# peterWon/GLoc3D

Hardware: AMD Instinct MI355X
Metric: localization queries/sec (kNN+top-20 reg), KITTI-00-sized DB (higher is better)
Workload: dtype f32

## Files before the change

gloc3d_amd/capi.py:

```python
import ctypes as C
import os

import numpy as np

HERE = os.path.dirname(os.path.abspath(__file__))
LIB_PATH = os.environ.get("GLOC3D_LIB_PATH") or os.path.join(HERE, "lib", "libgloc3d.so")

GLOC_OK = 0
ERR_NAMES = {1: "GLOC_ERR_INVALID", 2: "GLOC_ERR_HIP", 3: "GLOC_ERR_NOMEM", 4: "GLOC_ERR_NODEVICE",
             5: "GLOC_ERR_STATE"}
ALGO_AUTO, ALGO_EXACT, ALGO_MFMA, ALGO_MFMA_FP32 = 0, 1, 2, 3
KNN_OPT_ALGO, KNN_OPT_CANDIDATES, KNN_OPT_PROFILE = 1, 2, 3
REG_OPT_PROFILE, REG_OPT_NN_MODE, REG_OPT_NN_SRC_PER_LANE, REG_OPT_NN_JOB_GROUP, REG_OPT_TEMP_TARGET_INDEX = 1, 2, 3, 4, 5
REG_OPT_NN_SPLIT_HELPERS, REG_OPT_NN_SPLIT_THRESH, REG_OPT_NN_SUB_JOBS, REG_OPT_NN_HEAVY_THRESH, REG_OPT_SUB_BATCHES = 6, 7, 8, 9, 10
REG_OPT_NN_CHAIN = 11
REG_OPT_PAIRGRAPH_BUDGET = 12
REG_NN_CULLED, REG_NN_EXHAUSTIVE = 0, 1
NO_SCAN = 0xFFFFFFFF
SIZE_MAX = C.c_size_t(-1).value


class GlocError(RuntimeError):
    def __init__(self, code, msg):
        super().__init__(f"{ERR_NAMES.get(code, code)}: {msg}")
# ... 832 lines not shown
        perm, keys, kpos = np.empty(n, np.uint32), np.empty(n, np.uint32), np.empty(n, np.uint32)
        order2 = np.empty((n + 127) // 128, np.uint32)
        kd = C.c_int()
        check(f(self._h, int(scan_id), _np_ptr(perm), _np_ptr(keys), _np_ptr(kpos), _np_ptr(order2), C.byref(kd)))
        return dict(perm=perm, keys=keys, kpos=kpos, order2=order2, kd=bool(kd.value))

    def debug_boxes(self, scan_id, cs=2):
        f = lib().gloc_scan_store_debug_boxes
        f.restype = C.c_int
        f.argtypes = [C.c_void_p, C.c_uint32, C.c_int] + [C.c_void_p] * 9
        n = self.points(scan_id)
        nch = (n + 127) // 128
        n_pad, nsup, group = nch * 128, (nch + 63) // 64, 64 * int(cs)
        hb, hg = np.empty(6, np.uint32), np.empty(4, np.float32)
        box_lo, box_hi = np.empty((nch, 4), np.float32), np.empty((nch, 4), np.float32)
        sb2 = np.empty((n_pad // 32, 3, 4), np.float32)
        sup_lo, sup_hi = np.empty((nsup, 4), np.float32), np.empty((nsup, 4), np.float32)
        pad = np.empty((n_pad - n, 4), np.float32)
        order = np.empty((n + group - 1) // group if group else 0, np.uint32)
        check(f(self._h, int(scan_id), int(cs), *[_np_ptr(a) for a in (hb, hg, box_lo, box_hi, sb2, sup_lo, sup_hi, pad, order)]))
        return dict(lo=hb[:3].copy(), hi=hb[3:].copy(), ox=hg[0], oy=hg[1], oz=hg[2], inv_cell=hg[3], box_lo=box_lo,
                    box_hi=box_hi, sb2=sb2, sup_lo=sup_lo, sup_hi=sup_hi, pad=pad, order=order)

    def build_target_index_batch(self, scan_ids):
        ids = np.ascontiguousarray(scan_ids, np.uint32).reshape(-1)
        check(lib().gloc_scan_store_build_target_index_batch(self._h, _np_ptr(ids), ids.shape[0]))

    def release(self, scan_id):
        check(lib().gloc_scan_store_release(self._h, int(scan_id)))

    def clear(self):
        check(lib().gloc_scan_store_clear(self._h))

    def __len__(self):
        n = C.c_size_t()
        check(lib().gloc_scan_store_count(self._h, C.byref(n)))
        return n.value

    def bytes(self):
        a, b = C.c_size_t(), C.c_size_t()
        check(lib().gloc_scan_store_bytes(self._h, C.byref(a), C.byref(b)))
        return a.value, b.value

    def points(self, scan_id):
        n = C.c_size_t()
        check(lib().gloc_scan_store_points(self._h, int(scan_id), C.byref(n)))
# ... 1032 lines not shown
```

gloc3d_amd/csrc/nn_compact.hpp:

```cpp
#pragma once
#include <hip/hip_runtime.h>
#include <stdint.h>

#include <type_traits>

#include "lane_ops.hpp"
#include "reg_kernels.hpp"

namespace gloc {
namespace reg {

typedef float f32x2 __attribute__((ext_vector_type(2)));

#define GPTR(T) const T __attribute__((address_space(1)))*
#define CPTR(T) const T __attribute__((address_space(4)))*
constexpr float NN_NEAR = 1.0e-6f;
constexpr float NN_LB_SCALE = 0.999998f;
#ifndef GLOC_NN_THIN_MIN
#define GLOC_NN_THIN_MIN 32
#endif
#ifdef GLOC_NN_MARKS
#define NN_MARK(n) asm volatile("; NN_MARK " n)
#else
#define NN_MARK(n)
// ... 228 lines not shown
          uint32_t word = 0;
          if (parts > 1 && first + parts <= sp.hx) {
            for (uint32_t p = 0; p < parts; ++p) st_u32<true>(helper + first + p, g | (p << 20) | (parts << 24));
            word = (hid << 8) | parts;
          }
          st_u32<true>(plan + g, word);
        }
        run_h += 4u * (uint32_t)__popcll(b4) + 8u * (uint32_t)__popcll(b8);
        run_l += 2u * (uint32_t)__popcll(b2);
        run_gh += (uint32_t)__popcll(b4 | b8);
        run_gl += (uint32_t)__popcll(b2);
      }
    }
    for (uint32_t g = ng + (uint32_t)lane; g < n_groups; g += 64) st_u32<true>(plan + g, 0u);
  }
  if (pass + 1u < ch.n_pass) (void)chain_arrive(ch.ready + ((size_t)(pass + 1u) * n_jobs + job) * NN_CHAIN_PAD);
}


struct NnPos {
  uint32_t grp, slot, wgv;
  uint32_t role = 0, pass = 0, job = 0;
};

template <int CS, bool PAIRS, bool SPLIT = false ,
          bool WARM = false, bool HEAVY = false ,
          bool CHAIN = false >
__device__ __forceinline__ void nn_compact_body(
    const NnPos pos ,
    const Job* __restrict__ jobs, uint32_t n_jobs, uint32_t job_group, uint32_t n_wg , uint32_t subs,
    const CandState* __restrict__ states,
    const uint32_t* prev_corr , uint32_t* corr, float* __restrict__ d2out,
    f32x4* __restrict__ pairs, double* __restrict__ partials , uint32_t n_part,
    size_t ld, float gate2, NnSplit sp, NnHeavy hv, unsigned long long* __restrict__ stat_pairs ,
    const NnChain ch = NnChain{}) {
  constexpr int S = 64 * CS;
  constexpr int NSB = CH / SB;
  constexpr int SB_STRIDE = (SB / 2) * 8 + 8;
#ifndef GLOC_NN_QCAP
#define GLOC_NN_QCAP 256
#endif
#ifndef GLOC_NN_GRAN
#define GLOC_NN_GRAN 64
#endif
  constexpr int QCAP = GLOC_NN_QCAP;
  struct WaveLds {
// ... 53 lines not shown
    own_wave = false;
    if (gi >= J.n_groups) return;
  } else {
    const uint32_t wv = __builtin_amdgcn_readfirstlane(wg * NN_WPB + w);
    if (SPLIT && wv < sp.hx) {
      const uint32_t hw = ((CPTR(uint32_t))sp.helper)[(size_t)job * sp.hx + wv];
      if (hw == NN_NO_HELPER) return;
      gi = hw & 0xFFFFFu;
      part = (hw >> 20) & 15u;
      parts = hw >> 24;
      own_wave = false;
    } else {
      gi = wv - (SPLIT ? sp.hx : 0u);
    }
    if (gi >= J.n_groups) return;
    if constexpr (SPLIT) plan_word = ((CPTR(uint32_t))sp.plan)[(size_t)job * n_part + gi];
  }
  const unsigned long long pmask =
      !SPLIT || parts == 1 ? ~0ull : ((parts == 2 ? 0x5555555555555555ull : (parts == 4 ? 0x1111111111111111ull : (parts == 8 ? 0x0101010101010101ull : 0x0001000100010001ull))) << part);
  uint32_t w_cand = 0;
  struct IndexView {
    GPTR(f32x4) pts; GPTR(f32x4) box_lo; GPTR(f32x4) box_hi; GPTR(f32x4) sb2;
    GPTR(uint32_t) keys; GPTR(uint32_t) kpos; GPTR(uint32_t) inv; GPTR(ScanHeader) hdr;
    uint32_t n, nchunks;
    GPTR(f32x4) sup_lo; GPTR(f32x4) sup_hi;
    uint32_t nsup;
    CPTR(f32x4) cbox_lo; CPTR(f32x4) cbox_hi;
  };
  const ScanIndexDev ixg = J.tgt;
  const IndexView ix{(GPTR(f32x4))ixg.pts, (GPTR(f32x4))ixg.box_lo, (GPTR(f32x4))ixg.box_hi,
                     (GPTR(f32x4))ixg.sb2, (GPTR(uint32_t))ixg.keys, (GPTR(uint32_t))ixg.kpos,
                     (GPTR(uint32_t))ixg.inv, (GPTR(ScanHeader))ixg.hdr, ixg.n, ixg.nchunks,
                     (GPTR(f32x4))ixg.sup_lo, (GPTR(f32x4))ixg.sup_hi, ixg.nsup,
                     (CPTR(f32x4))ixg.box_lo, (CPTR(f32x4))ixg.box_hi};
  GPTR(f32x4) src4 = (GPTR(f32x4))J.src_pts;
  float T[12];
#pragma unroll
  for (int i = 0; i < 12; ++i) {
    if constexpr (CHAIN) T[i] = pos.pass ? ((CPTR(float))ch.Tp)[((size_t)pos.pass * n_jobs + job) * NN_CHAIN_T_STRIDE + i] : states[job].Tf[i];
    else T[i] = states[job].Tf[i];
  }

  const uint32_t wave_base = ((CPTR(uint32_t))J.src_order)[gi] * S;
  if constexpr (SPLIT && !HEAVY) {
    if (own_wave && (plan_word & 0xFFu) != 0u) return;
    hid = plan_word >> 8;
  }
  uint32_t n_processed = 0;
  unsigned long long n_items = 0;
  [[maybe_unused]] uint32_t n_rounds = 0;

  NN_MARK("load_xform_box");
  float px[CS], py[CS], pz[CS], best[CS];
  bool valid[CS];
  float wlo[3] = {3.4e38f, 3.4e38f, 3.4e38f}, whi[3] = {-3.4e38f, -3.4e38f, -3.4e38f};
// ... 30 lines not shown
  NN_MARK("upper_bounds");
  uint32_t b0s[CS];
#pragma unroll
  for (int s = 0; s < CS; ++s) {
    b0s[s] = 0;
    if (ix.n && pj[s] < ix.n) {
      const f32x4 t = pt[s];
      best[s] = dist2(px[s], py[s], pz[s], t.x, t.y, t.z);
      b0s[s] = pj[s] / (SB / 4);
    }
  }
  uint8_t tie0[CS];
#pragma unroll
  for (int s = 0; s < CS; ++s) tie0[s] = 0;
  if constexpr (HEAVY) {
#pragma unroll
    for (int s = 0; s < CS; ++s) {
      const unsigned long long k = hv.hkey[(size_t)hid * S + s * 64 + lane];
      best[s] = __uint_as_float((uint32_t)(k >> 32));
      b0s[s] = (uint32_t)k & 0x7FFFFFFFu;
      tie0[s] = (uint8_t)(((uint32_t)k >> 31) & 1u);
    }
  } else if constexpr (!WARM) {
#ifndef GLOC_NN_KEY_PROBES
#define GLOC_NN_KEY_PROBES 3
#endif
    constexpr int KP = GLOC_NN_KEY_PROBES;
    bool cold[CS];
    uint32_t key[CS], lo[CS], hi[CS];
    bool any = false;
#pragma unroll
    for (int s = 0; s < CS; ++s) {
      cold[s] = ix.n && !(pj[s] < ix.n);
      key[s] = morton_key(px[s], py[s], pz[s], ix.hdr->ox, ix.hdr->oy, ix.hdr->oz, ix.hdr->inv_cell);
      lo[s] = 0;
      hi[s] = cold[s] ? ix.n : 0u;
      any |= cold[s];
    }
    if (any) {
      for (;;) {
        bool go = false;
#pragma unroll
        for (int s = 0; s < CS; ++s) go |= hi[s] - lo[s] > (uint32_t)KP;
        if (!go) break;
        uint32_t pos[CS][KP], kv[CS][KP];
#pragma unroll
// ... 43 lines not shown
        for (int d = -2; d <= 2; ++d) {
          long long jj = (long long)lo[s] + d;
          jj = jj < 0 ? 0 : (jj >= (long long)ix.n ? (long long)ix.n - 1 : jj);
          pjj[s][d + 2] = !cold[s] ? 0u : (ix.kpos ? ix.kpos[jj] : (uint32_t)jj);
        }
      f32x4 tn[CS][5];
#pragma unroll
      for (int s = 0; s < CS; ++s)
#pragma unroll
        for (int d = 0; d < 5; ++d) tn[s][d] = ix.pts[pjj[s][d]];
#pragma unroll
      for (int s = 0; s < CS; ++s) {
        if (!cold[s]) continue;
#pragma unroll
        for (int d = 0; d < 5; ++d) {
          const float dd = dist2(px[s], py[s], pz[s], tn[s][d].x, tn[s][d].y, tn[s][d].z);
          if (dd < best[s]) {
            best[s] = dd;
            b0s[s] = pjj[s][d] / (SB / 4);
          }
        }
      }
    }
  }
#pragma unroll
  for (int s = 0; s < CS; ++s) {
    const uint32_t b0 = b0s[s];
    if (!valid[s]) best[s] = -1.f;
    const int slot = s * 64 + lane;
    L.src[slot] = f32x4{px[s], py[s], pz[s], 0.f};
    L.key[slot] = ((unsigned long long)__float_as_uint(best[s]) << 32) | b0;
    L.tie[slot] = tie0[s];
  }
  if (lane == 0) {
    L.src[S] = f32x4{0.f, 0.f, 0.f, 0.f};
    L.key[S] = (unsigned long long)__float_as_uint(-1.f) << 32;
  }
  constexpr float KS = SB2_INV_RANGE * SB2_INV_RANGE / NN_LB_SCALE;
  float bests[CS];
#pragma unroll
  for (int s = 0; s < CS; ++s) bests[s] = best[s] * KS;
  auto wave_max_best = [&]() {
    float m = -1.f;
#pragma unroll
    for (int s = 0; s < CS; ++s) m = fmaxf(m, bests[s]);
    return wave_minmax<true>(m);
// ... 244 lines not shown
            const unsigned long long k = L.key[slot];
            const unsigned long long old = __hip_atomic_fetch_min(hv.hkey + (size_t)hid * S + slot, k, __ATOMIC_RELAXED, __HIP_MEMORY_SCOPE_AGENT);
            const unsigned long long oldk = old & ~0x80000000ull;
            if (oldk < k) {
              const float od = __uint_as_float((uint32_t)(oldk >> 32)), md = __uint_as_float((uint32_t)(k >> 32));
              if ((old & 0x80000000ull) != 0ull || (md <= od * (1.0f + NN_NEAR) && ((uint32_t)oldk >> 2) != ((uint32_t)k >> 2))) L.tie[slot] = 1;
              L.key[slot] = oldk;
            }
          }
        }
      }
      bool changed = false;
#pragma unroll
      for (int s = 0; s < CS; ++s) {
        const float nb = __uint_as_float((uint32_t)(L.key[s * 64 + lane] >> 32));
        const float nbs = nb * KS;
        changed |= nbs < bests[s];
        bests[s] = nbs;
      }
      if (!WARM || wmax_s > 1.0e30f) {
        if (__builtin_amdgcn_ballot_w64(changed) != 0ull) wmax_s = wave_max_best();
      }
    };
  constexpr int NSEED = 4;
  uint32_t seed_c[NSEED];
#pragma unroll
  for (int k = 0; k < NSEED; ++k) seed_c[k] = 0xFFFFFFFFu;
  if constexpr (!WARM) {
    if (parts == 1 && ix.nchunks) {
      bool pend[CS];
      uint32_t sc[CS];
#pragma unroll
      for (int s = 0; s < CS; ++s) {
        sc[s] = b0s[s] / (uint32_t)(CH / (SB / 4));
        pend[s] = valid[s] && best[s] < 3.0e38f;
      }
      for (int k = 0; k < NSEED; ++k) {
        uint32_t c = 0xFFFFFFFFu;
#pragma unroll
        for (int s = CS - 1; s >= 0; --s) {
          const unsigned long long m = __builtin_amdgcn_ballot_w64(pend[s]);
          if (m) c = (uint32_t)__builtin_amdgcn_readlane((int)sc[s], __ffsll((long long)m) - 1);
        }
        if (c == 0xFFFFFFFFu) break;
        c = c < ix.nchunks ? c : ix.nchunks - 1;
#pragma unroll
        for (int j = 0; j < NSEED; ++j)
// ... 352 lines not shown
```

gloc3d_amd/csrc/scan_index.hpp:

```cpp
#pragma once
#include <hip/hip_runtime.h>
#include <stdint.h>

#include "math3.hpp"

namespace gloc {
namespace reg {

constexpr int CH = 128;
constexpr int SB = 16;
constexpr float SB2_RANGE = 64.f, SB2_INV_RANGE = 1.f / 64.f;

struct ScanHeader {
  float ox, oy, oz, inv_cell;
  uint32_t lo[3], hi[3];
  uint32_t pad_[6];
};
static_assert(sizeof(ScanHeader) == 64, "header is 64 bytes");

struct ScanIndexDev {
  const f32x4* pts;
  const f32x4* box_lo;
  const f32x4* box_hi;
  const f32x4* sb2;
  const uint32_t* kpos;
  const uint32_t* keys;
  const uint32_t* inv;
  const ScanHeader* hdr;
  const f32x4* sup_lo;
  const f32x4* sup_hi;
  uint32_t n, nchunks, nsup, pad_;
};

__host__ __device__ __forceinline__ uint32_t f2ord(float f) {
  const uint32_t u = __builtin_bit_cast(uint32_t, f);
  return (u & 0x80000000u) ? ~u : (u | 0x80000000u);
}
__host__ __device__ __forceinline__ float ord2f(uint32_t o) {
  const uint32_t u = (o & 0x80000000u) ? (o & 0x7FFFFFFFu) : ~o;
  return __builtin_bit_cast(float, u);
}

__host__ __device__ __forceinline__ bool finite_coord(float f) {
  return (__builtin_bit_cast(uint32_t, f) & 0x7F800000u) != 0x7F800000u;
}

}
}
```

gloc3d_amd/csrc/scan_store.hip:

```cpp
#include <algorithm>
#include <new>

#include "fpfh.hpp"
#include "scan_store.hpp"
#include "seg_sort.hpp"
#include <cmath>

#include "raycast_kernels.hpp"
#include "synth_kernels.hpp"

namespace gloc {
namespace reg {

constexpr int PACK_BLOCKS = 128;

struct ScanBuild {
  const float* in;
  ScanHeader* hdr;
  float* xyz;
  f32x4* pts;
  f32x4* lo;
  f32x4* hi;
  f32x4* sb2;
  f32x4* ulo;
// ... 264 lines not shown
                                    float sigma, uint64_t key, float* __restrict__ out) {
  const uint32_t i = blockIdx.x * blockDim.x + threadIdx.x;
  if (i >= n) return;
  float T[12];
#pragma unroll
  for (int k = 0; k < 12; ++k) T[k] = T12[k];
  float x, y, z;
  xform(T, xyz[3 * (size_t)i], xyz[3 * (size_t)i + 1], xyz[3 * (size_t)i + 2], x, y, z);
  const float nx = sigma * synth::rng_gauss(key, 3ull * i + 0);
  const float ny = sigma * synth::rng_gauss(key, 3ull * i + 1);
  const float nz = sigma * synth::rng_gauss(key, 3ull * i + 2);
  out[3 * (size_t)i + 0] = x + nx;
  out[3 * (size_t)i + 1] = y + ny;
  out[3 * (size_t)i + 2] = z + nz;
}

struct ScanKd {
  f32x4* pts;
  uint32_t* inv;
  uint32_t* kpos;
  uint32_t n, n_pad, levels;
  uint32_t off;
  uint32_t box_off;
  uint32_t pad_;
};

__global__ void kd_load_kernel(const ScanKd* __restrict__ ks, f32x4* __restrict__ p, uint32_t* __restrict__ h) {
  const ScanKd& k = ks[blockIdx.y];
  const uint32_t i = blockIdx.x * blockDim.x + threadIdx.x;
  if (i >= k.n) return;
  p[k.off + i] = k.pts[i];
  h[k.off + i] = i;
}

__global__ void kd_box_init_kernel(const ScanKd* __restrict__ ks, uint32_t level, uint32_t* __restrict__ box) {
  const ScanKd& k = ks[blockIdx.y];
  const uint32_t nd = blockIdx.x * blockDim.x + threadIdx.x;
  if (level >= k.levels || nd >= (1u << level)) return;
  uint32_t* b = box + k.box_off + 6 * (size_t)nd;
#pragma unroll
  for (int a = 0; a < 3; ++a) {
    b[a] = 0xFFFFFFFFu;
    b[3 + a] = 0u;
  }
}

__global__ __launch_bounds__(256) void kd_node_bbox_kernel(const ScanKd* __restrict__ ks, uint32_t level,
                                                           const f32x4* __restrict__ p_all, uint32_t* __restrict__ box) {
// ... 34 lines not shown
  if (lo[0] > hi[0] && lo[1] > hi[1] && lo[2] > hi[2]) return;
  uint32_t* o = box + k.box_off + 6 * (size_t)(first >> shift);
#pragma unroll
  for (int a = 0; a < 3; ++a) {
    atomicMin(o + a, lo[a]);
    atomicMax(o + 3 + a, hi[a]);
  }
}

__global__ void kd_keys_kernel(const ScanKd* __restrict__ ks, uint32_t level, const f32x4* __restrict__ p_all,
                               const uint32_t* __restrict__ box, unsigned long long* __restrict__ keys,
                               uint32_t* __restrict__ vals) {
  const ScanKd& k = ks[blockIdx.y];
  const uint32_t i = blockIdx.x * blockDim.x + threadIdx.x;
  if (i >= k.n) return;
  vals[k.off + i] = i;
  if (level >= k.levels) {
    keys[k.off + i] = i;
    return;
  }
  const uint32_t shift = 4 + k.levels - level;
  const uint32_t node = i >> shift;
  const uint32_t* b = box + k.box_off + 6 * (size_t)node;
  const float ex = b[0] <= b[3] ? ord2f(b[3]) - ord2f(b[0]) : -1.f, ey = b[1] <= b[4] ? ord2f(b[4]) - ord2f(b[1]) : -1.f,
              ez = b[2] <= b[5] ? ord2f(b[5]) - ord2f(b[2]) : -1.f;
  int axis = 0;
  float e = ex;
  if (ey > e) { axis = 1; e = ey; }
  if (ez > e) axis = 2;
  const f32x4 v = p_all[k.off + i];
  const float c = axis == 0 ? v.x : (axis == 1 ? v.y : v.z);
  keys[k.off + i] = ((unsigned long long)node << 32) | f2ord(c);
}

__global__ void kd_gather_kernel(const ScanKd* __restrict__ ks, const f32x4* __restrict__ p_in,
                                 const uint32_t* __restrict__ h_in, const uint32_t* __restrict__ perm,
                                 f32x4* __restrict__ p_out, uint32_t* __restrict__ h_out) {
  const ScanKd& k = ks[blockIdx.y];
  const uint32_t j = blockIdx.x * blockDim.x + threadIdx.x;
  if (j >= k.n) return;
  const uint32_t s = perm[k.off + j];
  p_out[k.off + j] = p_in[k.off + s];
  h_out[k.off + j] = h_in[k.off + s];
}

__global__ void kd_finish_kernel(const ScanKd* __restrict__ ks, const f32x4* __restrict__ p, const uint32_t* __restrict__ h) {
  const ScanKd& k = ks[blockIdx.y];
  const uint32_t j = blockIdx.x * blockDim.x + threadIdx.x;
  if (j >= k.n_pad) return;
  if (j >= k.n) {
    k.pts[j] = f32x4{NN_FAR, NN_FAR, NN_FAR, __uint_as_float(0xFFFFFFFFu)};
    return;
  }
  const f32x4 v = p[k.off + j];
  k.pts[j] = v;
  k.inv[__float_as_uint(v.w)] = j;
  k.kpos[h[k.off + j]] = j;
}

namespace {

struct Layout {
  size_t bytes, n1, np, c1, b1, u1, g1;
};
Layout layout_for(size_t n) {
  Layout L;
  const size_t nch = (n + CH - 1) / CH, nsup = (nch + 63) / 64;
  L.n1 = std::max<size_t>(n, 1);
  L.c1 = std::max<size_t>(nch, 1);
  L.np = L.c1 * CH;
  L.b1 = L.c1 * (CH / SB / 2) * 3;
  L.u1 = std::max<size_t>(nsup, 1);
  L.g1 = (L.n1 + 63) / 64;
  L.bytes = sizeof(ScanHeader) + sizeof(f32x4) * (L.np + 2 * L.c1 + L.b1 + 2 * L.u1) +
            sizeof(float) * 3 * L.n1 + sizeof(uint32_t) * (3 * L.n1 + 2 * L.g1 + 2);
  return L;
}

int take_block(gloc_scan_store* st, size_t bytes, void** out, size_t* cap) {
  auto it = st->free_blocks.lower_bound(bytes);
  if (it != st->free_blocks.end() && it->first <= bytes + bytes / 2 + (256u << 10)) {
    *out = it->second;
    *cap = it->first;
    st->cached_bytes -= it->first;
    st->free_blocks.erase(it);
    return GLOC_OK;
  }
  const size_t want = (bytes + (256u << 10) - 1) & ~(size_t)((256u << 10) - 1);
  hipError_t e = hipMalloc(out, want);
  if (e == hipErrorOutOfMemory && !st->free_blocks.empty()) {
    (void)hipGetLastError();
    (void)hipStreamSynchronize(st->stream);
    for (auto& kv : st->free_blocks) (void)hipFree(kv.second);
    st->free_blocks.clear();
    st->cached_bytes = 0;
    e = hipMalloc(out, want);
  }
  if (e != hipSuccess) {
// ... 125 lines not shown
  };
  size_t stage_floats = 0, total_pts = 0, total_grp = 0;
  uint32_t max_n = 0, max_np = 0, max_nch = 0, max_npairs = 0, max_nsup = 0;
  for (size_t i = 0; i < count; ++i) {
    DevScan s;
    s.n = n[i];
    const Layout L = layout_for(n[i]);
    const size_t nch = (n[i] + CH - 1) / CH, nsup = (nch + 63) / 64;
    if (int rc = take_block(st, L.bytes, &s.block, &s.block_bytes)) return fail(rc);
    ScanHeader* hdr = reinterpret_cast<ScanHeader*>(s.block);
    f32x4* p4 = reinterpret_cast<f32x4*>(hdr + 1);
    f32x4* lo = p4 + L.np;
    f32x4* hi = lo + L.c1;
    f32x4* sb2 = hi + L.c1;
    f32x4* ulo = sb2 + L.b1;
    f32x4* uhi = ulo + L.u1;
    s.xyz = reinterpret_cast<float*>(uhi + L.u1);
    uint32_t* keys = reinterpret_cast<uint32_t*>(s.xyz + 3 * L.n1);
    uint32_t* inv = keys + L.n1;
    s.order_base = inv + L.n1;
    s.order_g1 = L.g1;
    s.order = nullptr;
    s.kpos_mem = s.order_base + 2 * L.g1 + 2;
    s.idx = ScanIndexDev{p4, lo, hi, sb2, nullptr, keys, inv, hdr, ulo, uhi, (uint32_t)n[i], (uint32_t)nch,
                         (uint32_t)nsup, 0u};
    out[i] = s;
    made = i + 1;
    ScanBuild b = build_desc(s, L);
    b.stride = (uint32_t)stride;
    b.group = 128;
    b.n_groups = (uint32_t)((n[i] + b.group - 1) / b.group);
    b.order = s.order_of(2);
    b.key_off = (uint32_t)total_pts;
    b.grp_off = (uint32_t)total_grp;
    segs[i] = segsort::Seg{b.key_off, b.n};
    total_pts += (n[i] + 3) & ~(size_t)3;
    total_grp += b.n_groups;
    if (total_pts >= (1ull << 31)) {
      set_err("batch of scans too large (%zu points)", total_pts);
      return fail(GLOC_ERR_INVALID);
    }
    stage_floats += device_src ? 0 : stride * n[i];
    max_n = std::max(max_n, b.n);
    max_np = std::max(max_np, b.n_pad);
    max_nch = std::max(max_nch, b.nch);
    max_npairs = std::max(max_npairs, b.npairs);
// ... 59 lines not shown
    return fail(GLOC_ERR_HIP);
  }
  for (size_t i = 0; i < count; ++i) {
    out[i].order_built = n[i] ? (1u << 2) : 0u;
    out[i].live = true;
  }
  return GLOC_OK;
}

int store_make_scan(gloc_scan_store* st, const float* pts, size_t n, size_t stride, bool device_src, DevScan* out) {
  return store_make_scans(st, 1, &pts, &n, stride, device_src, out);
}

int store_build_target_indices(gloc_scan_store* st, DevScan* const* scans, size_t count) {
  hipStream_t q = st->stream;
  constexpr size_t MAX_BATCH_POINTS = size_t(8) << 20;
  size_t a = 0;
  while (a < count) {
    std::vector<ScanKd> hk;
    std::vector<ScanBuild> hb;
    std::vector<DevScan*> todo;
    std::vector<segsort::Seg> segs;
    size_t total = 0, box_words = 0, total_grp = 0;
    uint32_t max_n = 0, max_np = 0, max_levels = 0, max_nch = 0, max_npairs = 0, max_nsup = 0;
    size_t b = a;
    for (; b < count; ++b) {
      DevScan& s = *scans[b];
      if (s.kd) continue;
      if (s.n <= (size_t)SB) {
        s.kd = true;
        continue;
      }
      if (!todo.empty() && total + s.n > MAX_BATCH_POINTS) break;
      uint32_t L = 0;
      while (((size_t)SB << L) < s.n) ++L;
      const Layout lay = layout_for(s.n);
      ScanKd k{};
      k.pts = const_cast<f32x4*>(s.idx.pts);
      k.inv = const_cast<uint32_t*>(s.idx.inv);
      k.kpos = s.kpos_mem;
      k.n = (uint32_t)s.n;
      k.n_pad = (uint32_t)lay.np;
      k.levels = L;
      k.off = (uint32_t)total;
      k.box_off = (uint32_t)box_words;
      ScanBuild sb = build_desc(s, lay);
      sb.group = 128;
      sb.n_groups = (uint32_t)((s.n + 127) / 128);
      sb.order = s.order_of(2);
      sb.grp_off = (uint32_t)total_grp;
      segs.push_back(segsort::Seg{k.off, k.n});
      total += (s.n + 3) & ~(size_t)3;
      box_words += (size_t)6 << (L - 1);
      total_grp += sb.n_groups;
      max_n = std::max(max_n, k.n);
      max_np = std::max(max_np, k.n_pad);
      max_levels = std::max(max_levels, L);
      max_nch = std::max(max_nch, sb.nch);
      max_npairs = std::max(max_npairs, sb.npairs);
      max_nsup = std::max(max_nsup, sb.nsup);
      hk.push_back(k);
      hb.push_back(sb);
      todo.push_back(&s);
    }
    a = b;
    if (todo.empty()) continue;
    const uint32_t cnt = (uint32_t)todo.size();
    GLOC_TRY(st->kd_k0.ensure(sizeof(unsigned long long) * total, q));
// ... 13 lines not shown
    GLOC_HIP(hipMemcpyAsync(st->builds.p, hb.data(), sizeof(ScanBuild) * cnt, hipMemcpyHostToDevice, q));
    GLOC_HIP(hipMemcpyAsync(st->segs.p, segs.data(), sizeof(segsort::Seg) * cnt, hipMemcpyHostToDevice, q));
    const ScanKd* d_k = st->kd_desc.as<ScanKd>();
    f32x4* pp[2] = {st->kd_p0.as<f32x4>(), st->kd_p1.as<f32x4>()};
    uint32_t* hh[2] = {st->kd_h0.as<uint32_t>(), st->kd_h1.as<uint32_t>()};
    unsigned long long* kk[2] = {st->kd_k0.as<unsigned long long>(), st->kd_k1.as<unsigned long long>()};
    uint32_t* vv[2] = {st->kd_v0.as<uint32_t>(), st->kd_v1.as<uint32_t>()};
    const dim3 gpt((max_n + 255) / 256, cnt), gblk(((max_n + SB - 1) / SB + 255) / 256, cnt);
    std::vector<DevBuf> nrm_keep(cnt);
    for (uint32_t i = 0; i < cnt; ++i)
      if (todo[i]->nrm) {
        const uint32_t n = (uint32_t)todo[i]->n;
        GLOC_TRY(nrm_keep[i].ensure(12 * (size_t)n, q));
        GLOC_TRY(store_reorder_normals(q, todo[i]->idx.pts, n, todo[i]->nrm, nrm_keep[i].as<float>(), false));
      }
    std::vector<DevBuf> fpfh_keep(cnt);
    for (uint32_t i = 0; i < cnt; ++i)
      if (todo[i]->fpfh) {
        const uint32_t n = (uint32_t)todo[i]->n;
        GLOC_TRY(fpfh_keep[i].ensure(132 * (size_t)n, q));
        GLOC_TRY(gloc::fpfh::reorder_rows(q, todo[i]->idx.pts, n, todo[i]->fpfh, fpfh_keep[i].as<float>(), gloc::fpfh::FEAT_DIM, false));
      }
    hipLaunchKernelGGL(kd_load_kernel, gpt, dim3(256), 0, q, d_k, pp[0], hh[0]);
    int cur = 0;
    static_assert(SB == 16, "the node size arithmetic assumes 16-point leaves");
    for (uint32_t l = 0; l < max_levels; ++l) {
      hipLaunchKernelGGL(kd_box_init_kernel, dim3(((1u << l) + 255) / 256, cnt), dim3(256), 0, q, d_k, l, st->kd_box.as<uint32_t>());
      hipLaunchKernelGGL(kd_node_bbox_kernel, gblk, dim3(256), 0, q, d_k, l, pp[cur], st->kd_box.as<uint32_t>());
      hipLaunchKernelGGL(kd_keys_kernel, gpt, dim3(256), 0, q, d_k, l, pp[cur], st->kd_box.as<uint32_t>(), kk[0], vv[0]);
      const int r = segsort::sort_pairs<unsigned long long, 8>(q, kk[0], kk[1], vv[0], vv[1], st->segs.as<segsort::Seg>(), cnt,
                                                                max_n, 0, (int)(32 + l), st->sort_hist.as<uint32_t>());
      hipLaunchKernelGGL(kd_gather_kernel, gpt, dim3(256), 0, q, d_k, pp[cur], hh[cur], vv[r], pp[cur ^ 1], hh[cur ^ 1]);
      cur ^= 1;
    }
    hipLaunchKernelGGL(kd_finish_kernel, dim3((max_np + 255) / 256, cnt), dim3(256), 0, q, d_k, pp[cur], hh[cur]);
    launch_boxes(q, st->builds.as<ScanBuild>(), cnt, max_nch, max_npairs, max_nsup);
    for (uint32_t i = 0; i < cnt; ++i)
      if (todo[i]->nrm) GLOC_TRY(store_reorder_normals(q, todo[i]->idx.pts, (uint32_t)todo[i]->n, nrm_keep[i].as<float>(), todo[i]->nrm, true));
    for (uint32_t i = 0; i < cnt; ++i)
      if (todo[i]->fpfh)
        GLOC_TRY(gloc::fpfh::reorder_rows(q, todo[i]->idx.pts, (uint32_t)todo[i]->n, fpfh_keep[i].as<float>(), todo[i]->fpfh,
                                          gloc::fpfh::FEAT_DIM, true));
    GLOC_HIP(hipGetLastError());
    for (DevScan* s : todo) {
      s->idx.kpos = s->kpos_mem;
      s->kd = true;
      s->order_built = 0;
    }
    const int rc_orders = launch_orders(st, st->builds.as<ScanBuild>(), hb, cnt);
    if (rc_orders != GLOC_OK) {
      (void)hipStreamSynchronize(q);
      return rc_orders;
    }
    for (DevScan* s : todo) s->order_built = 1u << 2;
  }
  return GLOC_OK;
}

int store_build_target_index(gloc_scan_store* st, DevScan& s) {
  DevScan* p = &s;
  return store_build_target_indices(st, &p, 1);
}

int store_get(gloc_scan_store* st, uint32_t id, int cs, DevScan* out) {
  std::lock_guard<std::mutex> lk(st->mu);
  if (id >= st->scans.size() || !st->scans[id].live) {
    set_err("unknown scan id %u", id);
    return GLOC_ERR_INVALID;
// ... 330 lines not shown
  hipStream_t q = st->stream;
  if (perm) {
    std::vector<f32x4> p(s.n);
    GLOC_HIP(hipMemcpyAsync(p.data(), s.idx.pts, sizeof(f32x4) * s.n, hipMemcpyDeviceToHost, q));
    GLOC_HIP(hipStreamSynchronize(q));
    for (size_t i = 0; i < s.n; ++i) std::memcpy(&perm[i], reinterpret_cast<const char*>(&p[i]) + 12, 4);
  }
  if (keys) GLOC_HIP(hipMemcpyAsync(keys, s.idx.keys, sizeof(uint32_t) * s.n, hipMemcpyDeviceToHost, q));
  if (kpos) {
    if (s.idx.kpos) {
      GLOC_HIP(hipMemcpyAsync(kpos, s.idx.kpos, sizeof(uint32_t) * s.n, hipMemcpyDeviceToHost, q));
    } else {
      for (size_t i = 0; i < s.n; ++i) kpos[i] = (uint32_t)i;
    }
  }
  if (order2) {
    GLOC_TRY(store_build_order(st, s, 2));
    GLOC_HIP(hipMemcpyAsync(order2, s.order_of(2), sizeof(uint32_t) * ((s.n + 127) / 128), hipMemcpyDeviceToHost, q));
  }
  GLOC_HIP(hipStreamSynchronize(q));
  return GLOC_OK;
}

int gloc_scan_store_debug_boxes(gloc_scan_store* st, uint32_t scan_id, int cs, uint32_t* hdr_box, float* hdr_grid,
                                float* box_lo, float* box_hi, float* sb2, float* sup_lo, float* sup_hi, float* pad_pts,
                                uint32_t* order) {
  GLOC_REQUIRE(st, GLOC_ERR_INVALID, "null store");
  GLOC_REQUIRE(!order || cs == 1 || cs == 2 || cs == 4, GLOC_ERR_INVALID, "sources per lane must be 1, 2 or 4 (got %d)", cs);
  GLOC_HIP(hipSetDevice(st->device));
  std::lock_guard<std::mutex> lk(st->mu);
  GLOC_REQUIRE(scan_id < st->scans.size() && st->scans[scan_id].live, GLOC_ERR_INVALID, "unknown scan id %u", scan_id);
  DevScan& s = st->scans[scan_id];
  hipStream_t q = st->stream;
  if (hdr_box || hdr_grid) {
    ScanHeader h;
    GLOC_HIP(hipMemcpyAsync(&h, s.idx.hdr, sizeof(ScanHeader), hipMemcpyDeviceToHost, q));
    GLOC_HIP(hipStreamSynchronize(q));
    for (int a = 0; a < 3 && hdr_box; ++a) {
      hdr_box[a] = h.lo[a];
      hdr_box[3 + a] = h.hi[a];
    }
    if (hdr_grid) {
      hdr_grid[0] = h.ox;
      hdr_grid[1] = h.oy;
      hdr_grid[2] = h.oz;
      hdr_grid[3] = h.inv_cell;
// ... 37 lines not shown
```

gloc3d_amd/csrc/scan_store.hpp:

```cpp
#pragma once
#include <algorithm>
#include <atomic>
#include <map>
#include <mutex>
#include <vector>

#include "common.hpp"
#include "ground_normals.hpp"
#include "p2l.hpp"
#include "scan_index.hpp"

struct DevScan {
  void* block = nullptr;
  size_t block_bytes = 0;
  float* xyz = nullptr;
  size_t n = 0;
  gloc::reg::ScanIndexDev idx{};
  uint32_t* order_base = nullptr;
  uint32_t* order = nullptr;
  unsigned order_built = 0;
  uint32_t* kpos_mem = nullptr;
  size_t order_g1 = 0;
  uint32_t* order_of(int cs) const {
    return order_base + (cs == 1 ? 0 : cs == 2 ? order_g1 : order_g1 + (order_g1 + 1) / 2);
  }
  float* nrm = nullptr;
  gloc::Support nrm_sup;
  size_t nrm_bytes() const { return nrm ? 12 * n : 0; }
  float* fpfh = nullptr;
  gloc::Support fpfh_nsup, fpfh_fsup;
  size_t fpfh_bytes() const { return fpfh ? 132 * n : 0; }
  bool has_normals(const gloc::Support& ns) const { return nrm_sup == ns; }
  bool has_fpfh(const gloc::Support& ns, const gloc::Support& fs) const { return fpfh_nsup == ns && fpfh_fsup == fs && nrm_sup == ns; }
  uint32_t* kp = nullptr;
  float* kp_feat = nullptr;
  size_t kp_n = 0;
  bool kp_built = false;
  gloc_iss_params kp_prm{};
  size_t kp_bytes() const { return (kp ? 4 * kp_n : 0) + (kp_feat ? 132 * kp_n : 0); }
  bool has_keypoints(const gloc_iss_params& p) const {
    return kp_built && kp_prm.salient_radius == p.salient_radius && kp_prm.max_nn == p.max_nn && kp_prm.min_nn == p.min_nn &&
           kp_prm.non_max_radius == p.non_max_radius && kp_prm.gamma_21 == p.gamma_21 && kp_prm.gamma_32 == p.gamma_32;
  }
  bool live = false;
// ... 158 lines not shown
```

Measured before the change: 591.6.

## Seed cold NN search with a packed 3-level kd split table descent

Builds a compact table of kd-tree split planes, with three levels packed into each 32-byte record, while the target index is built. In the NN compaction kernel, cold sources walk this table to a leaf and take an initial best distance from a few leaf points, replacing the key-probe seeding path. The aim is a tighter initial bound for culling, at the cost of extra index memory, more build kernels, and dependent table loads per round. The seed count also becomes a compile-time macro.

```diff
diff --git a/gloc3d_amd/capi.py b/gloc3d_amd/capi.py
--- a/gloc3d_amd/capi.py
+++ b/gloc3d_amd/capi.py
@@ -878,6 +878,17 @@
         return dict(lo=hb[:3].copy(), hi=hb[3:].copy(), ox=hg[0], oy=hg[1], oz=hg[2], inv_cell=hg[3], box_lo=box_lo,
                     box_hi=box_hi, sb2=sb2, sup_lo=sup_lo, sup_hi=sup_hi, pad=pad, order=order)
 
+    def debug_kd_table(self, scan_id):
+        f = lib().gloc_scan_store_debug_kd_table
+        f.restype = C.c_int
+        f.argtypes = [C.c_void_p, C.c_uint32, C.POINTER(C.c_uint32), C.POINTER(C.c_size_t), C.c_void_p, C.c_size_t]
+        rounds, n_rec = C.c_uint32(), C.c_size_t()
+        check(f(self._h, int(scan_id), C.byref(rounds), C.byref(n_rec), None, 0))
+        rec = np.empty((n_rec.value, 8), np.uint32)
+        if n_rec.value:
+            check(f(self._h, int(scan_id), C.byref(rounds), C.byref(n_rec), _np_ptr(rec), rec.shape[0]))
+        return dict(rounds=int(rounds.value), split=rec[:, :7].copy().view(np.float32), axes=rec[:, 7].copy())
+
     def build_target_index_batch(self, scan_ids):
         ids = np.ascontiguousarray(scan_ids, np.uint32).reshape(-1)
         check(lib().gloc_scan_store_build_target_index_batch(self._h, _np_ptr(ids), ids.shape[0]))
diff --git a/gloc3d_amd/csrc/nn_compact.hpp b/gloc3d_amd/csrc/nn_compact.hpp
--- a/gloc3d_amd/csrc/nn_compact.hpp
+++ b/gloc3d_amd/csrc/nn_compact.hpp
@@ -274,6 +274,21 @@
   uint32_t grp, slot, wgv;
   uint32_t role = 0, pass = 0, job = 0;
 };
+
+__device__ __forceinline__ float kd_coord(uint32_t axis, float x, float y, float z) {
+  const float c01 = (axis & 1u) != 0u ? y : x;
+  return (axis & 2u) != 0u ? z : c01;
+}
+__device__ __forceinline__ uint32_t kd_record_child(f32x4 a, f32x4 b, float x, float y, float z) {
+  const uint32_t ax = __float_as_uint(b.w);
+  const bool g0 = kd_coord(ax, x, y, z) > a.x;
+  const float s1 = g0 ? a.z : a.y;
+  const bool g1 = kd_coord(ax >> (g0 ? 4 : 2), x, y, z) > s1;
+  const float s2l = g1 ? b.x : a.w, s2r = g1 ? b.z : b.y;
+  const uint32_t h2 = (g0 ? 2u : 0u) + (g1 ? 1u : 0u);
+  const bool g2 = kd_coord(ax >> (6u + 2u * h2), x, y, z) > (g0 ? s2r : s2l);
+  return h2 * 2u + (g2 ? 1u : 0u);
+}
 
 template <int CS, bool PAIRS, bool SPLIT = false ,
           bool WARM = false, bool HEAVY = false ,
@@ -373,6 +388,7 @@
   struct IndexView {
     GPTR(f32x4) pts; GPTR(f32x4) box_lo; GPTR(f32x4) box_hi; GPTR(f32x4) sb2;
     GPTR(uint32_t) keys; GPTR(uint32_t) kpos; GPTR(uint32_t) inv; GPTR(ScanHeader) hdr;
+    GPTR(KdRecord) kdt; uint32_t kd_rounds;
     uint32_t n, nchunks;
     GPTR(f32x4) sup_lo; GPTR(f32x4) sup_hi;
     uint32_t nsup;
@@ -381,7 +397,7 @@
   const ScanIndexDev ixg = J.tgt;
   const IndexView ix{(GPTR(f32x4))ixg.pts, (GPTR(f32x4))ixg.box_lo, (GPTR(f32x4))ixg.box_hi,
                      (GPTR(f32x4))ixg.sb2, (GPTR(uint32_t))ixg.keys, (GPTR(uint32_t))ixg.kpos,
-                     (GPTR(uint32_t))ixg.inv, (GPTR(ScanHeader))ixg.hdr, ixg.n, ixg.nchunks,
+                     (GPTR(uint32_t))ixg.inv, (GPTR(ScanHeader))ixg.hdr, (GPTR(KdRecord))ixg.kdt, ixg.kd_rounds, ixg.n, ixg.nchunks,
                      (GPTR(f32x4))ixg.sup_lo, (GPTR(f32x4))ixg.sup_hi, ixg.nsup,
                      (CPTR(f32x4))ixg.box_lo, (CPTR(f32x4))ixg.box_hi};
   GPTR(f32x4) src4 = (GPTR(f32x4))J.src_pts;
@@ -458,6 +474,69 @@
       tie0[s] = (uint8_t)(((uint32_t)k >> 31) & 1u);
     }
   } else if constexpr (!WARM) {
+   if (ix.kdt != nullptr) {
+    bool cold[CS];
+    uint32_t node[CS];
+#pragma unroll
+    for (int s = 0; s < CS; ++s) {
+      cold[s] = !(pj[s] < ix.n);
+      node[s] = 0;
+    }
+    const uint32_t R = ix.kd_rounds;
+    uint32_t first = 0;
+    for (uint32_t r = 0; r < R; ++r) {
+      f32x4 ra[CS], rb[CS];
+#pragma unroll
+      for (int s = 0; s < CS; ++s) {
+        GPTR(f32x4) rp = (GPTR(f32x4))(ix.kdt + (first + node[s]));
+        ra[s] = rp[0];
+        rb[s] = rp[1];
+      }
+#pragma unroll
+      for (int s = 0; s < CS; ++s) node[s] = node[s] * 8u + kd_record_child(ra[s], rb[s], px[s], py[s], pz[s]);
+      first += kd_level_records(ix.n, R, r);
+    }
+#ifndef GLOC_NN_LEAF_POINTS
+#define GLOC_NN_LEAF_POINTS 4
+#endif
+    constexpr int LP = GLOC_NN_LEAF_POINTS, LG = LP < 8 ? LP : 8;
+    static_assert(LP == 1 || LP == 4 || LP == 16, "1, 4 or 16 points of the leaf");
+    auto leaf_at = [](int i) { return LP == 16 ? i : (LP == 4 && i ? 4 * i + 1 : 0); };
+    typedef float f32x3 __attribute__((ext_vector_type(3)));
+    float mq[CS][4];
+#pragma unroll
+    for (int s = 0; s < CS; ++s)
+#pragma unroll
+      for (int q = 0; q < 4; ++q) mq[s][q] = 3.402823466e+38f;
+#pragma unroll
+    for (int i0 = 0; i0 < LP; i0 += LG) {
+      if (i0) __builtin_amdgcn_sched_barrier(0);
+      f32x3 t[CS][LG];
+#pragma unroll
+      for (int s = 0; s < CS; ++s)
+#pragma unroll
+        for (int u = 0; u < LG; ++u) t[s][u] = *(GPTR(f32x3))(ix.pts + ((size_t)node[s] * SB + leaf_at(i0 + u)));
+#pragma unroll
+      for (int s = 0; s < CS; ++s)
+#pragma unroll
+        for (int u = 0; u < LG; u += 2) {
+          const int v = u + 1 < LG ? u + 1 : u;
+          const f32x2 dx = f32x2{px[s], px[s]} - f32x2{t[s][u].x, t[s][v].x}, dy = f32x2{py[s], py[s]} - f32x2{t[s][u].y, t[s][v].y},
+                      dz = f32x2{pz[s], pz[s]} - f32x2{t[s][u].z, t[s][v].z};
+          const f32x2 d2 = __builtin_elementwise_fma(dz, dz, __builtin_elementwise_fma(dy, dy, dx * dx));
+          mq[s][leaf_at(i0 + u) / 4] = fminf(mq[s][leaf_at(i0 + u) / 4], d2.x);
+          mq[s][leaf_at(i0 + v) / 4] = fminf(mq[s][leaf_at(i0 + v) / 4], d2.y);
+        }
+    }
+#pragma unroll
+    for (int s = 0; s < CS; ++s) {
+      const float m = fminf(fminf(fminf(mq[s][0], mq[s][1]), mq[s][2]), mq[s][3]);
+      const uint32_t n0 = mq[s][0] != m ? 1u : 0u, n1 = n0 & (mq[s][1] != m ? 1u : 0u), n2 = n1 & (mq[s][2] != m ? 1u : 0u);
+      const bool take = cold[s] && m < best[s];
+      best[s] = take ? m : best[s];
+      b0s[s] = take ? node[s] * 4u + (n0 + n1 + n2) : b0s[s];
+    }
+   } else {
 #ifndef GLOC_NN_KEY_PROBES
 #define GLOC_NN_KEY_PROBES 3
 #endif
@@ -547,6 +626,7 @@
         }
       }
     }
+   }
   }
 #pragma unroll
   for (int s = 0; s < CS; ++s) {
@@ -837,7 +917,10 @@
         if (__builtin_amdgcn_ballot_w64(changed) != 0ull) wmax_s = wave_max_best();
       }
     };
-  constexpr int NSEED = 4;
+#ifndef GLOC_NN_SEEDS
+#define GLOC_NN_SEEDS 4
+#endif
+  constexpr int NSEED = GLOC_NN_SEEDS;
   uint32_t seed_c[NSEED];
 #pragma unroll
   for (int k = 0; k < NSEED; ++k) seed_c[k] = 0xFFFFFFFFu;
diff --git a/gloc3d_amd/csrc/scan_index.hpp b/gloc3d_amd/csrc/scan_index.hpp
--- a/gloc3d_amd/csrc/scan_index.hpp
+++ b/gloc3d_amd/csrc/scan_index.hpp
@@ -18,6 +18,8 @@
 };
 static_assert(sizeof(ScanHeader) == 64, "header is 64 bytes");
 
+struct KdRecord;
+
 struct ScanIndexDev {
   const f32x4* pts;
   const f32x4* box_lo;
@@ -29,8 +31,32 @@
   const ScanHeader* hdr;
   const f32x4* sup_lo;
   const f32x4* sup_hi;
-  uint32_t n, nchunks, nsup, pad_;
+  uint32_t n, nchunks, nsup;
+  uint32_t kd_rounds;
+  const KdRecord* kdt;
 };
+
+struct KdRecord {
+  float split[7];
+  uint32_t axes;
+};
+static_assert(sizeof(KdRecord) == 32, "one record is 32 bytes");
+
+__host__ __device__ __forceinline__ uint32_t kd_rounds_for(size_t n) {
+  uint32_t L = 0;
+  while (((size_t)SB << L) < n) ++L;
+  return (L + 2) / 3;
+}
+__host__ __device__ __forceinline__ uint32_t kd_level_records(uint32_t n, uint32_t R, uint32_t r) {
+  return ((n - 1u) >> (4u + 3u * (R - r))) + 1u;
+}
+__host__ __device__ __forceinline__ size_t kd_table_records(size_t n) {
+  if (n <= (size_t)SB) return 0;
+  const uint32_t R = kd_rounds_for(n);
+  size_t t = 0;
+  for (uint32_t r = 0; r < R; ++r) t += kd_level_records((uint32_t)n, R, r);
+  return t;
+}
 
 __host__ __device__ __forceinline__ uint32_t f2ord(float f) {
   const uint32_t u = __builtin_bit_cast(uint32_t, f);
diff --git a/gloc3d_amd/csrc/scan_store.hip b/gloc3d_amd/csrc/scan_store.hip
--- a/gloc3d_amd/csrc/scan_store.hip
+++ b/gloc3d_amd/csrc/scan_store.hip
@@ -310,8 +310,19 @@
   uint32_t n, n_pad, levels;
   uint32_t off;
   uint32_t box_off;
-  uint32_t pad_;
+  uint32_t kdt_records;
+  KdRecord* kdt;
 };
+
+__device__ __forceinline__ int kd_widest_axis(const uint32_t* b) {
+  const float ex = b[0] <= b[3] ? ord2f(b[3]) - ord2f(b[0]) : -1.f, ey = b[1] <= b[4] ? ord2f(b[4]) - ord2f(b[1]) : -1.f,
+              ez = b[2] <= b[5] ? ord2f(b[5]) - ord2f(b[2]) : -1.f;
+  int axis = 0;
+  float e = ex;
+  if (ey > e) { axis = 1; e = ey; }
+  if (ez > e) axis = 2;
+  return axis;
+}
 
 __global__ void kd_load_kernel(const ScanKd* __restrict__ ks, f32x4* __restrict__ p, uint32_t* __restrict__ h) {
   const ScanKd& k = ks[blockIdx.y];
@@ -392,12 +403,7 @@
   const uint32_t shift = 4 + k.levels - level;
   const uint32_t node = i >> shift;
   const uint32_t* b = box + k.box_off + 6 * (size_t)node;
-  const float ex = b[0] <= b[3] ? ord2f(b[3]) - ord2f(b[0]) : -1.f, ey = b[1] <= b[4] ? ord2f(b[4]) - ord2f(b[1]) : -1.f,
-              ez = b[2] <= b[5] ? ord2f(b[5]) - ord2f(b[2]) : -1.f;
-  int axis = 0;
-  float e = ex;
-  if (ey > e) { axis = 1; e = ey; }
-  if (ez > e) axis = 2;
+  const int axis = kd_widest_axis(b);
   const f32x4 v = p_all[k.off + i];
   const float c = axis == 0 ? v.x : (axis == 1 ? v.y : v.z);
   keys[k.off + i] = ((unsigned long long)node << 32) | f2ord(c);
@@ -414,6 +420,40 @@
   h_out[k.off + j] = h_in[k.off + s];
 }
 
+__global__ void kd_table_init_kernel(const ScanKd* __restrict__ ks) {
+  const ScanKd& k = ks[blockIdx.y];
+  const uint32_t t = blockIdx.x * blockDim.x + threadIdx.x;
+  if (t >= k.kdt_records) return;
+  KdRecord r;
+#pragma unroll
+  for (int h = 0; h < 7; ++h) r.split[h] = __builtin_inff();
+  r.axes = 0u;
+  k.kdt[t] = r;
+}
+
+__global__ void kd_planes_kernel(const ScanKd* __restrict__ ks, uint32_t level, const f32x4* __restrict__ p_all,
+                                 const uint32_t* __restrict__ box) {
+  const ScanKd& k = ks[blockIdx.y];
+  const uint32_t nd = blockIdx.x * blockDim.x + threadIdx.x;
+  if (level >= k.levels || nd >= (1u << level)) return;
+  const uint32_t size = (16u << k.levels) >> level;
+  const uint32_t mid = nd * size + size / 2;
+  if (mid >= k.n) return;
+  const int axis = kd_widest_axis(box + k.box_off + 6 * (size_t)nd);
+  const f32x4 v = p_all[k.off + mid - 1];
+  float c = axis == 0 ? v.x : (axis == 1 ? v.y : v.z);
+  if (c != c) c = (__float_as_uint(c) & 0x80000000u) ? -__builtin_inff() : __builtin_inff();
+  const uint32_t R = (k.levels + 2) / 3;
+  const uint32_t lam = level + 3 * R - k.levels;
+  const uint32_t r = lam / 3, j = lam % 3;
+  uint32_t first = 0;
+  for (uint32_t q = 0; q < r; ++q) first += kd_level_records(k.n, R, q);
+  const uint32_t h = (1u << j) - 1u + (nd & ((1u << j) - 1u));
+  KdRecord* rec = k.kdt + first + (nd >> j);
+  rec->split[h] = c;
+  atomicOr(&rec->axes, (uint32_t)axis << (2 * h));
+}
+
 __global__ void kd_finish_kernel(const ScanKd* __restrict__ ks, const f32x4* __restrict__ p, const uint32_t* __restrict__ h) {
   const ScanKd& k = ks[blockIdx.y];
   const uint32_t j = blockIdx.x * blockDim.x + threadIdx.x;
@@ -431,7 +471,7 @@
 namespace {
 
 struct Layout {
-  size_t bytes, n1, np, c1, b1, u1, g1;
+  size_t bytes, n1, np, c1, b1, u1, g1, kdt_off;
 };
 Layout layout_for(size_t n) {
   Layout L;
@@ -442,8 +482,9 @@
   L.b1 = L.c1 * (CH / SB / 2) * 3;
   L.u1 = std::max<size_t>(nsup, 1);
   L.g1 = (L.n1 + 63) / 64;
-  L.bytes = sizeof(ScanHeader) + sizeof(f32x4) * (L.np + 2 * L.c1 + L.b1 + 2 * L.u1) +
-            sizeof(float) * 3 * L.n1 + sizeof(uint32_t) * (3 * L.n1 + 2 * L.g1 + 2);
+  L.kdt_off = (sizeof(ScanHeader) + sizeof(f32x4) * (L.np + 2 * L.c1 + L.b1 + 2 * L.u1) + sizeof(float) * 3 * L.n1 +
+               sizeof(uint32_t) * (3 * L.n1 + 2 * L.g1 + 2) + 31) & ~(size_t)31;
+  L.bytes = L.kdt_off + sizeof(KdRecord) * kd_table_records(n);
   return L;
 }
 
@@ -615,6 +656,7 @@
     s.order_g1 = L.g1;
     s.order = nullptr;
     s.kpos_mem = s.order_base + 2 * L.g1 + 2;
+    s.kdt_mem = reinterpret_cast<KdRecord*>(static_cast<char*>(s.block) + L.kdt_off);
     s.idx = ScanIndexDev{p4, lo, hi, sb2, nullptr, keys, inv, hdr, ulo, uhi, (uint32_t)n[i], (uint32_t)nch,
                          (uint32_t)nsup, 0u};
     out[i] = s;
@@ -720,7 +762,7 @@
     std::vector<DevScan*> todo;
     std::vector<segsort::Seg> segs;
     size_t total = 0, box_words = 0, total_grp = 0;
-    uint32_t max_n = 0, max_np = 0, max_levels = 0, max_nch = 0, max_npairs = 0, max_nsup = 0;
+    uint32_t max_n = 0, max_np = 0, max_levels = 0, max_nch = 0, max_npairs = 0, max_nsup = 0, max_records = 0;
     size_t b = a;
     for (; b < count; ++b) {
       DevScan& s = *scans[b];
@@ -742,6 +784,9 @@
       k.levels = L;
       k.off = (uint32_t)total;
       k.box_off = (uint32_t)box_words;
+      k.kdt = s.kdt_mem;
+      k.kdt_records = (uint32_t)kd_table_records(s.n);
+      max_records = std::max(max_records, k.kdt_records);
       ScanBuild sb = build_desc(s, lay);
       sb.group = 128;
       sb.n_groups = (uint32_t)((s.n + 127) / 128);
@@ -801,6 +846,7 @@
         GLOC_TRY(gloc::fpfh::reorder_rows(q, todo[i]->idx.pts, n, todo[i]->fpfh, fpfh_keep[i].as<float>(), gloc::fpfh::FEAT_DIM, false));
       }
     hipLaunchKernelGGL(kd_load_kernel, gpt, dim3(256), 0, q, d_k, pp[0], hh[0]);
+    hipLaunchKernelGGL(kd_table_init_kernel, dim3((max_records + 255) / 256, cnt), dim3(256), 0, q, d_k);
     int cur = 0;
     static_assert(SB == 16, "the node size arithmetic assumes 16-point leaves");
     for (uint32_t l = 0; l < max_levels; ++l) {
@@ -811,6 +857,7 @@
                                                                 max_n, 0, (int)(32 + l), st->sort_hist.as<uint32_t>());
       hipLaunchKernelGGL(kd_gather_kernel, gpt, dim3(256), 0, q, d_k, pp[cur], hh[cur], vv[r], pp[cur ^ 1], hh[cur ^ 1]);
       cur ^= 1;
+      hipLaunchKernelGGL(kd_planes_kernel, dim3(((1u << l) + 255) / 256, cnt), dim3(256), 0, q, d_k, l, pp[cur], st->kd_box.as<uint32_t>());
     }
     hipLaunchKernelGGL(kd_finish_kernel, dim3((max_np + 255) / 256, cnt), dim3(256), 0, q, d_k, pp[cur], hh[cur]);
     launch_boxes(q, st->builds.as<ScanBuild>(), cnt, max_nch, max_npairs, max_nsup);
@@ -823,6 +870,8 @@
     GLOC_HIP(hipGetLastError());
     for (DevScan* s : todo) {
       s->idx.kpos = s->kpos_mem;
+      s->idx.kdt = s->kdt_mem;
+      s->idx.kd_rounds = kd_rounds_for(s->n);
       s->kd = true;
       s->order_built = 0;
     }
@@ -1199,6 +1248,23 @@
   return GLOC_OK;
 }
 
+int gloc_scan_store_debug_kd_table(gloc_scan_store* st, uint32_t scan_id, uint32_t* rounds, size_t* n_records, void* records,
+                                   size_t capacity_records) {
+  GLOC_REQUIRE(st && rounds && n_records, GLOC_ERR_INVALID, "null argument");
+  GLOC_HIP(hipSetDevice(st->device));
+  std::lock_guard<std::mutex> lk(st->mu);
+  GLOC_REQUIRE(scan_id < st->scans.size() && st->scans[scan_id].live, GLOC_ERR_INVALID, "unknown scan id %u", scan_id);
+  const DevScan& s = st->scans[scan_id];
+  *rounds = s.idx.kdt ? s.idx.kd_rounds : 0u;
+  *n_records = s.idx.kdt ? kd_table_records(s.n) : 0;
+  if (!records || !*n_records) return GLOC_OK;
+  GLOC_REQUIRE(capacity_records >= *n_records, GLOC_ERR_INVALID, "buffer holds %zu records, the table has %zu", capacity_records,
+               *n_records);
+  GLOC_HIP(hipMemcpyAsync(records, s.idx.kdt, sizeof(KdRecord) * *n_records, hipMemcpyDeviceToHost, st->stream));
+  GLOC_HIP(hipStreamSynchronize(st->stream));
+  return GLOC_OK;
+}
+
 int gloc_scan_store_debug_boxes(gloc_scan_store* st, uint32_t scan_id, int cs, uint32_t* hdr_box, float* hdr_grid,
                                 float* box_lo, float* box_hi, float* sb2, float* sup_lo, float* sup_hi, float* pad_pts,
                                 uint32_t* order) {
diff --git a/gloc3d_amd/csrc/scan_store.hpp b/gloc3d_amd/csrc/scan_store.hpp
--- a/gloc3d_amd/csrc/scan_store.hpp
+++ b/gloc3d_amd/csrc/scan_store.hpp
@@ -20,6 +20,7 @@
   uint32_t* order = nullptr;
   unsigned order_built = 0;
   uint32_t* kpos_mem = nullptr;
+  gloc::reg::KdRecord* kdt_mem = nullptr;
   size_t order_g1 = 0;
   uint32_t* order_of(int cs) const {
     return order_base + (cs == 1 ? 0 : cs == 2 ? order_g1 : order_g1 + (order_g1 + 1) / 2);
```

After: 606.3, median of 6. +2.5%, better.
